# mueller-franzes/medfusion

Hardware: AMD Instinct MI355X
Metric: images/sec at 256x256, 150 DDIM steps (DiffusionPipeline.sample incl. VAE decode) (higher is better)
Workload: dtype f32 (emulated: fp16 pairs -- 23-bit operands, and 23-bit STORAGE of the tensors between the UNet's conv blocks: they exist as fp16 pairs only)

## Files before the change

medfusion_amd/csrc/groupnorm.hip:

```cpp
#include "common.h"
#include <stdlib.h>
#include "gn_partial.h"

using namespace mf;

namespace {

__global__ __launch_bounds__(256) void gn_stats_final_kernel(const double* __restrict__ partial, float* __restrict__ stats, int NG, int G, int chunks,
                                                              double count, float eps) {
  const int t = blockIdx.x * blockDim.x + threadIdx.x;
  const int i = t >> 4, l = t & 15;
  double s = 0, q = 0;
  if (i < NG) {
    const int n = i / G, g = i - n * G;
    for (int c = l; c < chunks; c += 16) {
      const double* p = partial + (((long)n * chunks + c) * G + g) * 2;
      s += p[0]; q += p[1];
    }
  }
#pragma unroll
  for (int off = 8; off > 0; off >>= 1) {
    s += __shfl_xor(s, off, 64);
    q += __shfl_xor(q, off, 64);
  }
// ... 110 lines not shown
    *reinterpret_cast<float4*>(out + i * 4) = make_float4(e[0], e[1], e[2], e[3]);
    store_split4(sp.outs, i * 4, e[0], e[1], e[2], e[3], sc);
  }
}

struct GnChan {
  float mean[4], rstd[4], ga[4], be[4];
  float4 em;
};

__device__ __forceinline__ GnChan gn_chan_consts(const float* sm, const float* __restrict__ gamma, const float* __restrict__ beta,
                                                 const float* __restrict__ emb_row, int c, int cpg) {
  GnChan k;
  if (cpg % 4 == 0) {
    const int g = c / cpg;
#pragma unroll
    for (int i = 0; i < 4; ++i) { k.mean[i] = sm[2 * g]; k.rstd[i] = sm[2 * g + 1]; }
  } else {
#pragma unroll
    for (int i = 0; i < 4; ++i) { const int g = (c + i) / cpg; k.mean[i] = sm[2 * g]; k.rstd[i] = sm[2 * g + 1]; }
  }
  if (gamma) {
    const float4 ga = *reinterpret_cast<const float4*>(gamma + c), be = *reinterpret_cast<const float4*>(beta + c);
    k.ga[0] = ga.x; k.ga[1] = ga.y; k.ga[2] = ga.z; k.ga[3] = ga.w;
    k.be[0] = be.x; k.be[1] = be.y; k.be[2] = be.z; k.be[3] = be.w;
  } else {
#pragma unroll
    for (int i = 0; i < 4; ++i) { k.ga[i] = 1.f; k.be[i] = 0.f; }
  }
  k.em = emb_row ? *reinterpret_cast<const float4*>(emb_row + c) : make_float4(0.f, 0.f, 0.f, 0.f);
  return k;
}

template <bool SPLIT, int U>
__global__ __launch_bounds__(256) void gn_apply_part_kernel(const float* __restrict__ x, const double* __restrict__ partial, int parts, double count, float eps,
                                                            const float* __restrict__ gamma, const float* __restrict__ beta,
                                                            const float* __restrict__ residual, const float* __restrict__ emb, long emb_stride,
                                                            float* __restrict__ out, int HW, int C, int G, int act, const GnSplit sp) {
  __shared__ float sm[2 * 256 + 4];
  __shared__ double sd[2 * 256];
  const int n = blockIdx.y, tid = threadIdx.x;
  const int C4 = C >> 2, cpg = C / G;
  const unsigned per4 = (unsigned)HW * (unsigned)C4;
  const long base = (long)n * per4;
  constexpr unsigned SPAN = 256u * U;
  const unsigned step = gridDim.x * SPAN;
  const bool res_p = SPLIT && sp.res_pairs != nullptr;
  const bool res_f = !res_p && residual != nullptr;
  const bool fixed_c = (256 % C4) == 0;
  const float* emb_row = emb ? emb + (long)n * emb_stride : nullptr;

  float4 v[U], r[U];
  uint2 rh[U], rl[U];
  unsigned jw = blockIdx.x * SPAN;
#define GN_LOAD_ROUND()                                                                                                  \
  _Pragma("unroll") for (int u = 0; u < U; ++u) {                                                                        \
    const unsigned j = jw + 256u * u + tid;                                                                              \
    if (j < per4) {                                                                                                      \
      v[u] = *reinterpret_cast<const float4*>(x + (base + j) * 4);                                                       \
      if (res_p) {                                                                                                       \
        const long e = (base + j) * 4;                                                                                   \
        const uint2* g_ = reinterpret_cast<const uint2*>(reinterpret_cast<const char*>(sp.res_pairs) + (e >> 3) * 32 + ((e >> 2) & 1) * 8); \
        rh[u] = g_[0]; rl[u] = g_[2];                            \
      } else if (res_f) r[u] = *reinterpret_cast<const float4*>(residual + (base + j) * 4);                              \
    }                                                                                                                    \
  }
// ... 37 lines not shown
  }
  GnChan kc = gn_chan_consts(sm, gamma, beta, emb_row, fixed_c ? (tid % C4) * 4 : 0, cpg);

  while (jw < per4) {
#pragma unroll
    for (int u = 0; u < U; ++u) {
      const unsigned j = jw + 256u * u + tid;
      if (j < per4) {
        if (!fixed_c) kc = gn_chan_consts(sm, gamma, beta, emb_row, (int)(j % (unsigned)C4) * 4, cpg);
        float e[4] = {v[u].x, v[u].y, v[u].z, v[u].w};
#pragma unroll
        for (int k = 0; k < 4; ++k) {
          float t = (e[k] - kc.mean[k]) * kc.rstd[k];
          if (gamma) t = t * kc.ga[k] + kc.be[k];
          if (act == 1) t = swish_apply(t);
          e[k] = t;
        }
        if (res_p) {
          const sf_f16x2 h0 = __builtin_bit_cast(sf_f16x2, rh[u].x), h1 = __builtin_bit_cast(sf_f16x2, rh[u].y),
                         l0 = __builtin_bit_cast(sf_f16x2, rl[u].x), l1 = __builtin_bit_cast(sf_f16x2, rl[u].y);
          e[0] += ((float)h0[0] + (float)l0[0] * kLoInv) * rsc; e[1] += ((float)h0[1] + (float)l0[1] * kLoInv) * rsc;
          e[2] += ((float)h1[0] + (float)l1[0] * kLoInv) * rsc; e[3] += ((float)h1[1] + (float)l1[1] * kLoInv) * rsc;
        } else if (res_f) { e[0] += r[u].x; e[1] += r[u].y; e[2] += r[u].z; e[3] += r[u].w; }
        if (emb) { e[0] += kc.em.x; e[1] += kc.em.y; e[2] += kc.em.z; e[3] += kc.em.w; }
        if (!SPLIT || out) *reinterpret_cast<float4*>(out + (base + j) * 4) = make_float4(e[0], e[1], e[2], e[3]);
        if (SPLIT) store_split4<false>(sp.outs, (base + j) * 4, e[0], e[1], e[2], e[3], sc);
      }
    }
    jw += step;
    if (jw < per4) GN_LOAD_ROUND()
  }
#undef GN_LOAD_ROUND
}

__global__ __launch_bounds__(256) void maxabs_kernel(const float* __restrict__ x, float* __restrict__ partial, long per_sample4) {
  const int n = blockIdx.y;
  const float4* p = reinterpret_cast<const float4*>(x) + (long)n * per_sample4;
  float m = 0.f;
  for (long i = (long)blockIdx.x * blockDim.x + threadIdx.x; i < per_sample4; i += (long)gridDim.x * blockDim.x) {
    const float4 v = p[i];
    m = fmaxf(fmaxf(m, fmaxf(fabsf(v.x), fabsf(v.y))), fmaxf(fabsf(v.z), fabsf(v.w)));
  }
  m = wave_max(m);
  if ((threadIdx.x & 63) == 0) partial[((long)n * gridDim.x + blockIdx.x) * 4 + (threadIdx.x >> 6)] = m;
}

__global__ __launch_bounds__(64) void bound_finalize_kernel(const float* __restrict__ partial, float* __restrict__ bound, int slots) {
  const int n = blockIdx.x;
  float m = 0.f;
  for (int i = threadIdx.x; i < slots; i += 64) m = fmaxf(m, partial[(long)n * slots + i]);
  m = wave_max(m);
  if (threadIdx.x == 0) bound[n] = m;
}

}

extern "C" {

size_t mf_gn_stats_workspace_bytes(int N, int HW, int C, int G) {
  if (N <= 0 || HW <= 0 || G <= 0) return 0;
  return (size_t)N * stats_chunks(HW) * G * 2 * sizeof(double);
}

int mf_gn_stats_f32(const float* x, float* stats, void* workspace, size_t workspace_bytes, int N, int HW, int C, int G, float eps,
                    void* stream) {
  MF_REQUIRE(x && stats && N > 0 && HW > 0 && C > 0 && G > 0, MF_EINVAL, "gn_stats: bad args");
// ... 58 lines not shown
                                  int C, int G, int act, void* stream) {
  return mf_gn_apply_from_partials_pairs_f32(x, gn_partial, parts, eps, gamma, beta, residual, nullptr, emb, emb_stride, out, out_split, res_bound,
                                             res_bound_slots, res_nslots, emb_bound, bconst, out_bound, N, HW, C, G, act, stream);
}

int mf_gn_apply_from_partials_pairs_f32(const float* x, const double* gn_partial, int parts, float eps, const float* gamma, const float* beta,
                                        const float* residual, const void* residual_pairs, const float* emb, int64_t emb_stride, float* out,
                                        void* out_split, const float* res_bound, const float* res_bound_slots, int res_nslots,
                                        const float* emb_bound, float bconst, float* out_bound, int N, int HW, int C, int G, int act, void* stream) {
  MF_REQUIRE(x && (out || out_split) && gn_partial && parts > 0 && N > 0 && N <= 65535 && HW > 0 && C > 0, MF_EINVAL, "gn_apply_from_partials: bad args");
  MF_REQUIRE(!residual_pairs || (!residual && out_split && res_bound), MF_EINVAL,
             "gn_apply_from_partials: a residual given as fp16 pairs needs out_split and the res_bound that scaled it, and excludes the fp32 residual");
  MF_REQUIRE(G > 0 && G <= 256 && C % G == 0 && C % 4 == 0, MF_EUNSUPPORTED, "gn_apply_from_partials: C=%d G=%d (C %% 4 == 0, C %% G == 0, G <= 256)", C, G);
  MF_REQUIRE(!out_split || (C % 8 == 0 && out_bound), MF_EUNSUPPORTED, "gn_apply_from_partials: the fp16-pair output needs C %% 8 == 0 and out_bound");
  MF_REQUIRE(!out_split || !residual || res_bound || (res_bound_slots && res_nslots > 0), MF_EINVAL,
             "gn_apply_from_partials: the fp16-pair output needs res_bound (or res_bound_slots) with a residual");
  MF_REQUIRE(!out_split || !emb || emb_bound, MF_EINVAL, "gn_apply_from_partials: the fp16-pair output needs emb_bound with an embedding");
  MF_REQUIRE((gamma == nullptr) == (beta == nullptr), MF_EINVAL, "gn_apply_from_partials: gamma/beta must both be given or both NULL");
  MF_REQUIRE(!emb || emb_stride % 4 == 0, MF_EUNSUPPORTED, "gn_apply_from_partials: emb_stride must be a multiple of 4");
  hipStream_t s = (hipStream_t)stream;
  const long per4 = (long)HW * (C / 4);
  const double nelem = (double)N * HW * C;
  ProfScope ps(MF_FAM_GN_APPLY, s, 8.0 * nelem, 4.0 * nelem * (1 + (out ? 1 : 0) + (residual || residual_pairs ? 1 : 0) + (out_split ? 1 : 0)));
  MF_REQUIRE(per4 < (1L << 31), MF_EUNSUPPORTED, "gn_apply_from_partials: %ld float4 per sample", per4);
  const long total_blocks = ((long)N * per4 + 255) / 256;
  static const int force_u = [] { const char* e = getenv("MF_GN_U"); const int v = e ? atoi(e) : 0; return (v == 1 || v == 2 || v == 4) ? v : 0; }();
  const int U = force_u ? force_u : total_blocks >= 4 * 1024 ? 4 : total_blocks >= 2 * 1024 ? 2 : 1;
  long bps = (per4 + 256 * U - 1) / (256 * U);
  static const int per_cu = [] { const char* e = getenv("MF_GN_BLOCKS_PER_CU"); const int v = e ? atoi(e) : 8; return v < 1 ? 1 : v > 32 ? 32 : v; }();
  const long cap = (256 * per_cu + N - 1) / N;
  if (bps > cap) bps = cap;
  const GnSplit sp{out_split, nullptr, res_bound, emb_bound, bconst, out_bound, res_bound ? nullptr : res_bound_slots, res_nslots, residual_pairs};
  const double count = (double)HW * (C / G);
#define GN_PART_LAUNCH(SPLIT_, U_)                                                                                                          \
  MF_LAUNCH((gn_apply_part_kernel<SPLIT_, U_>), dim3((int)bps, N), dim3(256), 0, s, x, gn_partial, parts, count, eps, gamma, beta, residual, emb, \
            (long)emb_stride, out, HW, C, G, act, sp)
  if (out_split) {
    if (U == 4) GN_PART_LAUNCH(true, 4); else if (U == 2) GN_PART_LAUNCH(true, 2); else GN_PART_LAUNCH(true, 1);
  } else {
    if (U == 4) GN_PART_LAUNCH(false, 4); else if (U == 2) GN_PART_LAUNCH(false, 2); else GN_PART_LAUNCH(false, 1);
  }
#undef GN_PART_LAUNCH
  return check_launch("gn_apply_from_partials");
}

int mf_maxabs_rows_slots(int64_t per_row) {
  const long p4 = per_row / 4;
  int blocks = (int)((p4 + 1023) / 1024);
  if (blocks > 64) blocks = 64;
  if (blocks < 1) blocks = 1;
  return blocks * 4;
}

int mf_maxabs_rows_f32(const float* x, float* partial, float* bound, int N, int64_t per_row, void* stream) {
  MF_REQUIRE(x && partial && N > 0 && per_row > 0 && per_row % 4 == 0 && N <= 65535, MF_EINVAL, "maxabs_rows: bad args (per_row %% 4 == 0)");
  hipStream_t s = (hipStream_t)stream;
  ProfScope ps(MF_FAM_MISC, s, 0, 4.0 * N * (double)per_row);
  const int slots = mf_maxabs_rows_slots(per_row);
  MF_LAUNCH(maxabs_kernel, dim3(slots / 4, N), dim3(256), 0, s, x, partial, (long)(per_row / 4));
  int rc = check_launch("maxabs_rows");
  if (rc || !bound) return rc;
  MF_LAUNCH(bound_finalize_kernel, dim3(N), dim3(64), 0, s, partial, bound, slots);
  return check_launch("bound_finalize");
}

int mf_bound_finalize_f32(const float* partial, float* bound, int N, int slots, void* stream) {
  MF_REQUIRE(partial && bound && N > 0 && slots > 0, MF_EINVAL, "bound_finalize: bad args");
  ProfScope ps(MF_FAM_MISC, (hipStream_t)stream, 0, 4.0 * N * slots);
  MF_LAUNCH(bound_finalize_kernel, dim3(N), dim3(64), 0, (hipStream_t)stream, partial, bound, slots);
  return check_launch("bound_finalize");
}


int mf_gn_partial_parts(int HW) { return HW > 0 ? stats_chunks(HW) : 0; }

// ... 24 lines not shown
```

medfusion_amd/csrc/split_f16.h:

```cpp
#pragma once
#include <hip/hip_runtime.h>

namespace mf {

typedef float sf_f32x4 __attribute__((ext_vector_type(4)));
typedef unsigned int sf_u32x4 __attribute__((ext_vector_type(4)));
typedef unsigned int sf_u32x2 __attribute__((ext_vector_type(2)));
typedef _Float16 sf_f16x2 __attribute__((ext_vector_type(2)));

constexpr float kLoScale = 2048.f, kLoInv = 1.f / 2048.f, kF16Max = 65504.f;

__device__ __forceinline__ int scale_exp_of(float bound) {
  const int e = (int)((__float_as_uint(bound) >> 23) & 0xffu) - 127;
  const int s = e - 14;
  return s < -100 ? -100 : (s > 100 ? 100 : s);
}
__device__ __forceinline__ float exp2i(int s) { return __uint_as_float((unsigned)(127 + s) << 23); }

__device__ __forceinline__ float clamp_f16_range(float a) {
  const float c = __builtin_fminf(__builtin_fmaxf(a, -kF16Max), kF16Max);
  return __builtin_fabsf(a) <= 3.4028234663852886e38f ? c : a;
}
template <bool CLAMP = true>
__device__ __forceinline__ void split2_f16(float a, float b, unsigned& hi, unsigned& lo) {
  if (CLAMP) {
    a = clamp_f16_range(a);
    b = clamp_f16_range(b);
  }
  const _Float16 ha = (_Float16)a, hb = (_Float16)b;
  const float ra = (a - (float)ha) * kLoScale, rb = (b - (float)hb) * kLoScale;
  const sf_f16x2 h = {ha, hb}, l = {(_Float16)ra, (_Float16)rb};
  hi = __builtin_bit_cast(unsigned, h);
  lo = __builtin_bit_cast(unsigned, l);
}
template <bool CLAMP = true>
__device__ __forceinline__ void split8_f16(const sf_f32x4 v0, const sf_f32x4 v1, sf_u32x4& hi, sf_u32x4& lo) {
  const float a0 = v0[0], a1 = v0[1], a2 = v0[2], a3 = v0[3], b0 = v1[0], b1 = v1[1], b2 = v1[2], b3 = v1[3];
  unsigned h0, h1, h2, h3, l0, l1, l2, l3;
  split2_f16<CLAMP>(a0, a1, h0, l0);
  split2_f16<CLAMP>(a2, a3, h1, l1);
  split2_f16<CLAMP>(b0, b1, h2, l2);
  split2_f16<CLAMP>(b2, b3, h3, l3);
  hi = sf_u32x4{h0, h1, h2, h3};
// ... 29 lines not shown
```

medfusion_amd/csrc/winograd.h:

```cpp
#pragma once
#include "common.h"
#include "split_f16.h"

namespace mfw {
using namespace mf;
typedef float wf32x4 __attribute__((ext_vector_type(4)));

__global__ __launch_bounds__(256) void wino_pack_weight_kernel(const float* __restrict__ w, float* __restrict__ u, long n) {
  const long i = (long)blockIdx.x * 256 + threadIdx.x;
  if (i >= n) return;
  double g[3][3], t[4][3];
#pragma unroll
  for (int r = 0; r < 3; ++r)
#pragma unroll
    for (int c = 0; c < 3; ++c) g[r][c] = (double)w[i * 9 + r * 3 + c];
#pragma unroll
  for (int c = 0; c < 3; ++c) {
    t[0][c] = g[0][c];
    t[1][c] = 0.5 * (g[0][c] + g[1][c] + g[2][c]);
    t[2][c] = 0.5 * (g[0][c] - g[1][c] + g[2][c]);
    t[3][c] = g[2][c];
  }
#pragma unroll
  for (int r = 0; r < 4; ++r) {
// ... 7 lines not shown

__device__ __forceinline__ float4 wino_load_pairs4(const void* pairs, long e) {
  const uint2* g = reinterpret_cast<const uint2*>(reinterpret_cast<const char*>(pairs) + (e >> 3) * 32 + ((e >> 2) & 1) * 8);
  const uint2 h = g[0], l = g[2];
  const sf_f16x2 h0 = __builtin_bit_cast(sf_f16x2, h.x), h1 = __builtin_bit_cast(sf_f16x2, h.y), l0 = __builtin_bit_cast(sf_f16x2, l.x),
                 l1 = __builtin_bit_cast(sf_f16x2, l.y);
  return make_float4((float)h0[0] + (float)l0[0] * kLoInv, (float)h0[1] + (float)l0[1] * kLoInv, (float)h1[0] + (float)l1[0] * kLoInv,
                     (float)h1[1] + (float)l1[1] * kLoInv);
}

__device__ __forceinline__ void wino_bt_d_b(float* d) {
#pragma unroll
  for (int c = 0; c < 4; ++c) {
    const float d0 = d[c], d1 = d[4 + c], d2 = d[8 + c], d3 = d[12 + c];
    d[c] = d0 - d2; d[4 + c] = d1 + d2; d[8 + c] = d2 - d1; d[12 + c] = d1 - d3;
  }
#pragma unroll
  for (int r = 0; r < 4; ++r) {
    const float t0 = d[4 * r], t1 = d[4 * r + 1], t2 = d[4 * r + 2], t3 = d[4 * r + 3];
    d[4 * r] = t0 - t2; d[4 * r + 1] = t1 + t2; d[4 * r + 2] = t2 - t1; d[4 * r + 3] = t1 - t3;
  }
}

__global__ __launch_bounds__(256) void wino_input_kernel(const void* __restrict__ xs, const float* __restrict__ xbound, void* __restrict__ vs,
                                                          float* __restrict__ vbound, int N, int H, int W, int C) {
  const int C4 = C >> 2, TW = W >> 1, T = (H >> 1) * TW;
  const long total = (long)N * T * C4, stride = (long)gridDim.x * 256;
  const long plane = (long)N * T * C;
  for (long i = (long)blockIdx.x * 256 + threadIdx.x; i < total; i += stride) {
    const int c4 = (int)(i % C4);
    const long r = i / C4;
    const int tile = (int)(r % T), n = (int)(r / T);
    const int ty = tile / TW, tx = tile - ty * TW;
    const float b = xbound ? xbound[n] : 0.f;
    const float vb = 4.f * b;
    const float f = xbound ? exp2i(scale_exp_of(b)) * exp2i(-scale_exp_of(vb)) : 1.f;
    float d[4][16];
#pragma unroll
    for (int py = 0; py < 4; ++py)
#pragma unroll
      for (int px = 0; px < 4; ++px) {
        const int y = 2 * ty - 1 + py, x = 2 * tx - 1 + px;
        float4 v = make_float4(0.f, 0.f, 0.f, 0.f);
        if ((unsigned)y < (unsigned)H && (unsigned)x < (unsigned)W) v = wino_load_pairs4(xs, (((long)n * H + y) * W + x) * C + c4 * 4);
        d[0][4 * py + px] = v.x; d[1][4 * py + px] = v.y; d[2][4 * py + px] = v.z; d[3][4 * py + px] = v.w;
      }
#pragma unroll
    for (int k = 0; k < 4; ++k) wino_bt_d_b(d[k]);
    const long e0 = ((long)n * T + tile) * C + c4 * 4;
#pragma unroll
    for (int k = 0; k < 16; ++k) store_split4<true>(vs, (long)k * plane + e0, d[0][k], d[1][k], d[2][k], d[3][k], f);
    if (vbound && tile == 0 && c4 == 0) {
#pragma unroll
      for (int k = 0; k < 16; ++k) vbound[k * N + n] = vb;
    }
  }
}

__global__ __launch_bounds__(256) void wino_input_f32_kernel(const float* __restrict__ x, float* __restrict__ v, int N, int H, int W, int C) {
  const int C4 = C >> 2, TW = W >> 1, T = (H >> 1) * TW;
  const long total = (long)N * T * C4, stride = (long)gridDim.x * 256;
  const long plane = (long)N * T * C;
  for (long i = (long)blockIdx.x * 256 + threadIdx.x; i < total; i += stride) {
    const int c4 = (int)(i % C4);
    const long r = i / C4;
    const int tile = (int)(r % T), n = (int)(r / T);
    const int ty = tile / TW, tx = tile - ty * TW;
    float d[4][16];
#pragma unroll
    for (int py = 0; py < 4; ++py)
#pragma unroll
      for (int px = 0; px < 4; ++px) {
        const int y = 2 * ty - 1 + py, xx = 2 * tx - 1 + px;
        float4 q = make_float4(0.f, 0.f, 0.f, 0.f);
        if ((unsigned)y < (unsigned)H && (unsigned)xx < (unsigned)W) q = *reinterpret_cast<const float4*>(x + (((long)n * H + y) * W + xx) * C + c4 * 4);
        d[0][4 * py + px] = q.x; d[1][4 * py + px] = q.y; d[2][4 * py + px] = q.z; d[3][4 * py + px] = q.w;
      }
#pragma unroll
    for (int k = 0; k < 4; ++k) wino_bt_d_b(d[k]);
// ... 91 lines not shown
  void* out_pairs;
  float* out_bound;
  void* out_wino;
  float* wino_bound;
  int N, H, W, C, G, act;
  float eps, bconst;
  int v_nt;
  int v_f32;
  int xcd_map;
};

__device__ __forceinline__ float wino_pair_round(float a) {
  const _Float16 h = (_Float16)a;
  const _Float16 l = (_Float16)((a - (float)h) * kLoScale);
  return (float)h + (float)l * kLoInv;
}

__global__ __launch_bounds__(256) void wino_tail_kernel(const WinoTailP p) {
  extern __shared__ __attribute__((aligned(16))) float ys[];
  __shared__ double sd[8];
  __shared__ float sf[8];
  const int tid = threadIdx.x, lane = tid & 63, wave = tid >> 6;
  int lin = blockIdx.x;
  if (p.xcd_map) {
    const int total = p.G * p.N, q = total >> 3, r = total & 7, xcd = lin & 7, within = lin >> 3;
    lin = (xcd < r ? xcd * (q + 1) : r * (q + 1) + (xcd - r) * q) + within;
  }
  const int g = lin % p.G, n = lin / p.G;
  const int C = p.C, cpg = C / p.G, cq = cpg >> 2, c0 = g * cpg;
  const int H = p.H, W = p.W, HW = H * W, TW = W >> 1, T = (H >> 1) * TW;
  const long plane = (long)p.N * T * C;
  const int c4 = tid % cq;
  constexpr int RJ = 4;
  uint2 rph[RJ], rpl[RJ];
  float4 rpf[RJ];
#pragma unroll
  for (int j = 0; j < RJ; ++j) {
    rph[j] = make_uint2(0u, 0u); rpl[j] = make_uint2(0u, 0u); rpf[j] = make_float4(0.f, 0.f, 0.f, 0.f);
    const int it = tid + 256 * j;
    if (it < HW * cq) {
      const long eo = ((long)n * HW + it / cq) * C + c0 + c4 * 4;
      if (p.res_pairs) {
        const uint2* gp = reinterpret_cast<const uint2*>(reinterpret_cast<const char*>(p.res_pairs) + (eo >> 3) * 32 + ((eo >> 2) & 1) * 8);
        rph[j] = gp[0]; rpl[j] = gp[2];
      } else if (p.res_f32) {
        rpf[j] = *reinterpret_cast<const float4*>(p.res_f32 + eo);
      }
    }
  }
  const float4 b4 = p.bias ? *reinterpret_cast<const float4*>(p.bias + c0 + c4 * 4) : make_float4(0.f, 0.f, 0.f, 0.f);
  double s = 0, q = 0;
  for (int it = tid; it < T * cq; it += 256) {
    const int t = it / cq;
    const float* src = p.m + ((long)n * T + t) * C + c0 + c4 * 4;
    float4 v[16];
#pragma unroll
    for (int k = 0; k < 16; ++k) v[k] = *reinterpret_cast<const float4*>(src + (long)k * plane);
    float4 o[4];
#pragma unroll
    for (int e = 0; e < 4; ++e) {
      float mm[16];
#pragma unroll
      for (int k = 0; k < 16; ++k) mm[k] = e == 0 ? v[k].x : e == 1 ? v[k].y : e == 2 ? v[k].z : v[k].w;
      float a0[4], a1[4];
#pragma unroll
      for (int c = 0; c < 4; ++c) {
        a0[c] = (mm[c] + mm[4 + c]) + mm[8 + c];
        a1[c] = (mm[4 + c] - mm[8 + c]) - mm[12 + c];
      }
      const float be = e == 0 ? b4.x : e == 1 ? b4.y : e == 2 ? b4.z : b4.w;
      const float y00 = ((a0[0] + a0[1]) + a0[2]) + be, y01 = ((a0[1] - a0[2]) - a0[3]) + be;
      const float y10 = ((a1[0] + a1[1]) + a1[2]) + be, y11 = ((a1[1] - a1[2]) - a1[3]) + be;
      if (e == 0) { o[0].x = y00; o[1].x = y01; o[2].x = y10; o[3].x = y11; }
      if (e == 1) { o[0].y = y00; o[1].y = y01; o[2].y = y10; o[3].y = y11; }
      if (e == 2) { o[0].z = y00; o[1].z = y01; o[2].z = y10; o[3].z = y11; }
      if (e == 3) { o[0].w = y00; o[1].w = y01; o[2].w = y10; o[3].w = y11; }
    }
    const int ty = t / TW, tx = t - ty * TW;
    float* dst = ys + ((2 * ty) * W + 2 * tx) * cpg + c4 * 4;
    *reinterpret_cast<float4*>(dst) = o[0];
    *reinterpret_cast<float4*>(dst + cpg) = o[1];
    *reinterpret_cast<float4*>(dst + W * cpg) = o[2];
    *reinterpret_cast<float4*>(dst + W * cpg + cpg) = o[3];
    float s1 = 0.f, s2 = 0.f;
#pragma unroll
    for (int j = 0; j < 4; ++j) {
      s1 += (o[j].x + o[j].y) + (o[j].z + o[j].w);
      s2 = fmaf(o[j].x, o[j].x, s2); s2 = fmaf(o[j].y, o[j].y, s2); s2 = fmaf(o[j].z, o[j].z, s2); s2 = fmaf(o[j].w, o[j].w, s2);
    }
    s += (double)s1;
    q += (double)s2;
  }
#pragma unroll
  for (int off = 32; off > 0; off >>= 1) {
    s += __shfl_xor(s, off, 64);
    q += __shfl_xor(q, off, 64);
  }
  if (lane == 0) { sd[wave] = s; sd[4 + wave] = q; }
  if (p.res_slots) {
    float mx = 0.f;
    for (int i = tid; i < p.res_nslots; i += 256) mx = fmaxf(mx, p.res_slots[(long)n * p.res_nslots + i]);
    mx = wave_max(mx);
    if (lane == 0) sf[wave] = mx;
  }
  __syncthreads();
  const double S = ((sd[0] + sd[1]) + sd[2]) + sd[3], Q = ((sd[4] + sd[5]) + sd[6]) + sd[7];
  const double count = (double)HW * cpg;
  const double mean_d = S / count;
  double var = Q / count - mean_d * mean_d;
  if (var < 0) var = 0;
  const float mean = (float)mean_d, rstd = (float)(1.0 / sqrt(var + (double)p.eps));
  const float rb = p.res_slots ? fmaxf(fmaxf(sf[0], sf[1]), fmaxf(sf[2], sf[3])) : (p.res_bound ? p.res_bound[n] : 0.f);
  const float ob = p.bconst + rb + (p.emb_bound ? p.emb_bound[n] : 0.f);
  const float osc = exp2i(-scale_exp_of(ob));
  const float rsc = p.res_pairs ? exp2i(scale_exp_of(p.res_bound[n])) : 1.f;
  const float vb = 4.f * ob;
  if (g == 0) {
    if (tid == 0 && p.out_bound) p.out_bound[n] = ob;
    if (tid < 16 && p.wino_bound) p.wino_bound[tid * p.N + n] = vb;
  }
  float ga[4] = {1.f, 1.f, 1.f, 1.f}, be[4] = {0.f, 0.f, 0.f, 0.f};
  if (p.gamma) {
    const float4 g4 = *reinterpret_cast<const float4*>(p.gamma + c0 + c4 * 4), e4 = *reinterpret_cast<const float4*>(p.beta + c0 + c4 * 4);
    ga[0] = g4.x; ga[1] = g4.y; ga[2] = g4.z; ga[3] = g4.w;
    be[0] = e4.x; be[1] = e4.y; be[2] = e4.z; be[3] = e4.w;
  }
  const float4 em = p.emb ? *reinterpret_cast<const float4*>(p.emb + (long)n * p.emb_stride + c0 + c4 * 4) : make_float4(0.f, 0.f, 0.f, 0.f);
  const bool keep = p.out_wino != nullptr;
  auto pairs_to_f4 = [](uint2 h, uint2 l) {
    const sf_f16x2 h0 = __builtin_bit_cast(sf_f16x2, h.x), h1 = __builtin_bit_cast(sf_f16x2, h.y), l0 = __builtin_bit_cast(sf_f16x2, l.x),
                   l1 = __builtin_bit_cast(sf_f16x2, l.y);
    return make_float4((float)h0[0] + (float)l0[0] * kLoInv, (float)h0[1] + (float)l0[1] * kLoInv, (float)h1[0] + (float)l1[0] * kLoInv,
                       (float)h1[1] + (float)l1[1] * kLoInv);
  };
#define WINO_TAIL_ELEMENT(IT, RES_EXPR_PAIRS, RES_EXPR_F32)                                                            \
  {                                                                                                                   \
    const int pix = (IT) / cq;                                                                                        \
    float* yp = ys + pix * cpg + c4 * 4;                                                                              \
    const float4 v = *reinterpret_cast<const float4*>(yp);                                                            \
    float e[4] = {v.x, v.y, v.z, v.w};                                                                                \
    _Pragma("unroll") for (int k = 0; k < 4; ++k) {                                                                   \
      float t = (e[k] - mean) * rstd;                                                                                 \
      if (p.gamma) t = t * ga[k] + be[k];                                                                             \
      if (p.act == 1) t = swish_apply(t);                                                                             \
      e[k] = t;                                                                                                       \
    }                                                                                                                 \
    const long eo = ((long)n * HW + pix) * C + c0 + c4 * 4;                                                           \
    if (p.res_pairs) {                                                                                                \
      const float4 r = RES_EXPR_PAIRS;                                                                                \
      e[0] += r.x * rsc; e[1] += r.y * rsc; e[2] += r.z * rsc; e[3] += r.w * rsc;                                     \
    } else if (p.res_f32) {                                                                                           \
      const float4 r = RES_EXPR_F32;                                                                                  \
      e[0] += r.x; e[1] += r.y; e[2] += r.z; e[3] += r.w;                                                             \
    }                                                                                                                 \
    if (p.emb) { e[0] += em.x; e[1] += em.y; e[2] += em.z; e[3] += em.w; }                                            \
    if (p.out_f32) *reinterpret_cast<float4*>(p.out_f32 + eo) = make_float4(e[0], e[1], e[2], e[3]);                  \
    if (p.out_pairs) store_split4<false>(p.out_pairs, eo, e[0], e[1], e[2], e[3], osc);    \
    if (keep) *reinterpret_cast<float4*>(yp) = p.v_f32 ? make_float4(e[0], e[1], e[2], e[3])                                                                     \
                                                       : make_float4(wino_pair_round(e[0] * osc), wino_pair_round(e[1] * osc), wino_pair_round(e[2] * osc), wino_pair_round(e[3] * osc)); \
  }
#pragma unroll
  for (int j = 0; j < RJ; ++j) {
    const int it = tid + 256 * j;
    if (it < HW * cq) WINO_TAIL_ELEMENT(it, pairs_to_f4(rph[j], rpl[j]), rpf[j])
  }
  for (int it = tid + 256 * RJ; it < HW * cq; it += 256) WINO_TAIL_ELEMENT(it, wino_load_pairs4(p.res_pairs, eo), *reinterpret_cast<const float4*>(p.res_f32 + eo))
#undef WINO_TAIL_ELEMENT
  if (!keep) return;
  __syncthreads();
  const float f = exp2i(scale_exp_of(ob)) * exp2i(-scale_exp_of(vb));
  for (int it = tid; it < T * cq; it += 256) {
    const int t = it / cq, ty = t / TW, tx = t - ty * TW;
    float d[4][16];
#pragma unroll
    for (int py = 0; py < 4; ++py)
#pragma unroll
      for (int px = 0; px < 4; ++px) {
        const int y = 2 * ty - 1 + py, x = 2 * tx - 1 + px;
        float4 v = make_float4(0.f, 0.f, 0.f, 0.f);
        if ((unsigned)y < (unsigned)H && (unsigned)x < (unsigned)W) v = *reinterpret_cast<const float4*>(ys + (y * W + x) * cpg + c4 * 4);
        d[0][4 * py + px] = v.x; d[1][4 * py + px] = v.y; d[2][4 * py + px] = v.z; d[3][4 * py + px] = v.w;
      }
#pragma unroll
    for (int k = 0; k < 4; ++k) wino_bt_d_b(d[k]);
    const long e0 = ((long)n * T + t) * C + c0 + c4 * 4;
    if (p.v_f32) {
#pragma unroll
      for (int k = 0; k < 16; ++k)
        __builtin_nontemporal_store(wf32x4{d[0][k], d[1][k], d[2][k], d[3][k]}, reinterpret_cast<wf32x4*>(reinterpret_cast<float*>(p.out_wino) + (long)k * plane + e0));
    } else if (p.v_nt) {
#pragma unroll
      for (int k = 0; k < 16; ++k) store_split4<true, true>(p.out_wino, (long)k * plane + e0, d[0][k], d[1][k], d[2][k], d[3][k], f);
    } else {
#pragma unroll
      for (int k = 0; k < 16; ++k) store_split4<true>(p.out_wino, (long)k * plane + e0, d[0][k], d[1][k], d[2][k], d[3][k], f);
    }
  }
}

}
```

Baseline: 40.57.

## Hoist and prefetch residual/param loads in GroupNorm apply and Winograd tail kernels

Adds a new code path, on by default, in the GroupNorm apply kernel, the Winograd input transform and the fused GN/Winograd tail. It issues the activation, residual, gamma/beta, embedding and bound loads unconditionally before the statistics reduction, using a zero buffer in place of null pointers, and pins them in registers with asm barriers. The tail residual loop is software-pipelined one element ahead, with output-mode specialisation, and fixed-channel handling becomes a template parameter. A lighter LDS-only barrier replaces __syncthreads. The aim is to overlap global-memory latency with the reduction and remove branchy dependent loads, at the cost of more register pressure and some redundant loads.

```diff
diff --git a/medfusion_amd/csrc/groupnorm.hip b/medfusion_amd/csrc/groupnorm.hip
--- a/medfusion_amd/csrc/groupnorm.hip
+++ b/medfusion_amd/csrc/groupnorm.hip
@@ -166,6 +166,163 @@
   return k;
 }
 
+#if MF_PASS_CHAIN == 2
+__device__ __forceinline__ GnChan gn_chan_consts_any(const float* sm, const float* __restrict__ gamma, const float* __restrict__ beta,
+                                                     const float* __restrict__ emb_row, int c, int cpg) {
+  GnChan k;
+  const float4 ga = *reinterpret_cast<const float4*>(gamma ? gamma + c : kZeros8), be = *reinterpret_cast<const float4*>(gamma ? beta + c : kZeros8);
+  k.em = *reinterpret_cast<const float4*>(emb_row ? emb_row + c : kZeros8);
+  k.ga[0] = ga.x; k.ga[1] = ga.y; k.ga[2] = ga.z; k.ga[3] = ga.w;
+  k.be[0] = be.x; k.be[1] = be.y; k.be[2] = be.z; k.be[3] = be.w;
+  if (cpg % 4 == 0) {
+    const int g = c / cpg;
+#pragma unroll
+    for (int i = 0; i < 4; ++i) { k.mean[i] = sm[2 * g]; k.rstd[i] = sm[2 * g + 1]; }
+  } else {
+#pragma unroll
+    for (int i = 0; i < 4; ++i) { const int g = (c + i) / cpg; k.mean[i] = sm[2 * g]; k.rstd[i] = sm[2 * g + 1]; }
+  }
+  return k;
+}
+
+template <bool SPLIT, int U, bool FIXED_C>
+__global__ __launch_bounds__(256) void gn_apply_part_kernel(const float* __restrict__ x, const double* __restrict__ partial, int parts, double count, float eps,
+                                                            const float* __restrict__ gamma, const float* __restrict__ beta,
+                                                            const float* __restrict__ residual, const float* __restrict__ emb, long emb_stride,
+                                                            float* __restrict__ out, int HW, int C, int G, int act, const GnSplit sp) {
+  __shared__ float sm[2 * 256 + 4];
+  __shared__ double sd[2 * 256];
+  const int n = blockIdx.y, tid = threadIdx.x;
+  const int C4 = C >> 2, cpg = C / G;
+  const unsigned per4 = (unsigned)HW * (unsigned)C4;
+  const long base = (long)n * per4;
+  constexpr unsigned SPAN = 256u * U;
+  const unsigned step = gridDim.x * SPAN;
+  const bool res_p = SPLIT && sp.res_pairs != nullptr;
+  const bool res_f = !res_p && residual != nullptr;
+  constexpr bool fixed_c = FIXED_C;
+  const float* emb_row = emb ? emb + (long)n * emb_stride : nullptr;
+  const int PPT = 256 / G, g = tid % G, kk = tid / G;
+
+  const double* rp0 = partial + (((long)n * parts + min(kk, parts - 1)) * G + g) * 2;
+  const double rec_s = rp0[0], rec_q = rp0[1];
+  float rbv = 0.f, ebv = 0.f, sl0 = 0.f;
+  if (SPLIT) {
+    rbv = *(sp.res_bound ? sp.res_bound + n : kZeros8);
+    ebv = *(sp.emb_bound ? sp.emb_bound + n : kZeros8);
+    sl0 = *((sp.res_slots && sp.res_nslots > 0) ? sp.res_slots + (long)n * sp.res_nslots + min(tid, sp.res_nslots - 1) : kZeros8);
+  }
+  const int cfix = fixed_c ? (tid % C4) * 4 : 0;
+  float4 g4 = *reinterpret_cast<const float4*>(gamma ? gamma + cfix : kZeros8), e4 = *reinterpret_cast<const float4*>(gamma ? beta + cfix : kZeros8);
+  float4 em4 = *reinterpret_cast<const float4*>(emb_row ? emb_row + cfix : kZeros8);
+  const char* const rbase = res_p ? reinterpret_cast<const char*>(sp.res_pairs) : res_f ? reinterpret_cast<const char*>(residual) : reinterpret_cast<const char*>(kZeros8);
+  const int rhalf = res_p ? 16 : 8;
+  float4 v[U];
+  uint2 ra[U], rb[U];
+  unsigned jw = blockIdx.x * SPAN;
+#define GN_LOAD_ROUND()                                                                                                  \
+  _Pragma("unroll") for (int u = 0; u < U; ++u) {                                                                        \
+    const long e = (base + min(jw + 256u * u + tid, per4 - 1u)) * 4;                                                     \
+    v[u] = *reinterpret_cast<const float4*>(x + e);                                                                      \
+    const char* q_ = rbase + (res_p ? (e >> 3) * 32 + ((e >> 2) & 1) * 8 : res_f ? e * 4 : 0L);                          \
+    ra[u] = *reinterpret_cast<const uint2*>(q_);                                                                         \
+    rb[u] = *reinterpret_cast<const uint2*>(q_ + rhalf);    \
+  }
+  GN_LOAD_ROUND()
+
+  {
+    double s = 0, q = 0;
+    if (kk < PPT) {
+      if (kk < parts) { s += rec_s; q += rec_q; }
+      for (int k = kk + PPT; k < parts; k += PPT) {
+        const double* p = partial + (((long)n * parts + k) * G + g) * 2;
+        s += p[0]; q += p[1];
+      }
+    }
+    sd[tid] = s; sd[256 + tid] = q;
+  }
+  if (SPLIT && sp.res_slots) {
+    float m = fmaxf(0.f, sl0);
+    for (int i = tid + 256; i < sp.res_nslots; i += 256) m = fmaxf(m, sp.res_slots[(long)n * sp.res_nslots + i]);
+    m = wave_max(m);
+    if ((tid & 63) == 0) sm[2 * 256 + (tid >> 6)] = m;
+  }
+  MF_LDS_BARRIER();
+  if (tid < G) {
+    double s = sd[tid], q = sd[256 + tid];
+    for (int k2 = 1; k2 < PPT; ++k2) { s += sd[k2 * G + tid]; q += sd[256 + k2 * G + tid]; }
+    const double mean = s / count;
+    double var = q / count - mean * mean;
+    if (var < 0) var = 0;
+    sm[2 * tid] = (float)mean;
+    sm[2 * tid + 1] = (float)(1.0 / sqrt(var + (double)eps));
+  }
+  MF_LDS_BARRIER();
+  float sc = 1.f, rsc = 1.f, obound = 0.f;
+  if (SPLIT) {
+    const float rbd = sp.res_slots ? fmaxf(fmaxf(sm[512], sm[513]), fmaxf(sm[514], sm[515])) : rbv;
+    obound = sp.bconst + rbd + ebv;
+    sc = exp2i(-scale_exp_of(obound));
+    if (res_p) rsc = exp2i(scale_exp_of(rbv));
+  }
+  GnChan kc;
+  {
+    if (cpg % 4 == 0) {
+      const int gq = cfix / cpg;
+#pragma unroll
+      for (int i = 0; i < 4; ++i) { kc.mean[i] = sm[2 * gq]; kc.rstd[i] = sm[2 * gq + 1]; }
+    } else {
+#pragma unroll
+      for (int i = 0; i < 4; ++i) { const int gq = (cfix + i) / cpg; kc.mean[i] = sm[2 * gq]; kc.rstd[i] = sm[2 * gq + 1]; }
+    }
+    asm volatile("" : "+v"(g4.x), "+v"(g4.y), "+v"(g4.z), "+v"(g4.w), "+v"(e4.x), "+v"(e4.y), "+v"(e4.z), "+v"(e4.w), "+v"(em4.x), "+v"(em4.y), "+v"(em4.z), "+v"(em4.w));
+    kc.ga[0] = g4.x; kc.ga[1] = g4.y; kc.ga[2] = g4.z; kc.ga[3] = g4.w;
+    kc.be[0] = e4.x; kc.be[1] = e4.y; kc.be[2] = e4.z; kc.be[3] = e4.w;
+    kc.em = em4;
+  }
+
+  for (;;) {
+#pragma unroll
+    for (int u = 0; u < U; ++u)
+      asm volatile("" : "+v"(v[u].x), "+v"(v[u].y), "+v"(v[u].z), "+v"(v[u].w), "+v"(ra[u].x), "+v"(ra[u].y), "+v"(rb[u].x), "+v"(rb[u].y));
+#pragma unroll
+    for (int u = 0; u < U; ++u) {
+      const unsigned j = jw + 256u * u + tid;
+      if (j < per4) {
+        if (!fixed_c) {
+          kc = gn_chan_consts_any(sm, gamma, beta, emb_row, (int)(j % (unsigned)C4) * 4, cpg);
+          asm volatile("" : "+v"(kc.ga[0]), "+v"(kc.ga[1]), "+v"(kc.ga[2]), "+v"(kc.ga[3]), "+v"(kc.be[0]), "+v"(kc.be[1]), "+v"(kc.be[2]), "+v"(kc.be[3]),
+                            "+v"(kc.em.x), "+v"(kc.em.y), "+v"(kc.em.z), "+v"(kc.em.w));
+        }
+        float e[4] = {v[u].x, v[u].y, v[u].z, v[u].w};
+#pragma unroll
+        for (int k = 0; k < 4; ++k) {
+          float t = (e[k] - kc.mean[k]) * kc.rstd[k];
+          if (gamma) t = t * kc.ga[k] + kc.be[k];
+          if (act == 1) t = swish_apply(t);
+          e[k] = t;
+        }
+        if (res_p) {
+          const sf_f16x2 h0 = __builtin_bit_cast(sf_f16x2, ra[u].x), h1 = __builtin_bit_cast(sf_f16x2, ra[u].y),
+                         l0 = __builtin_bit_cast(sf_f16x2, rb[u].x), l1 = __builtin_bit_cast(sf_f16x2, rb[u].y);
+          e[0] += ((float)h0[0] + (float)l0[0] * kLoInv) * rsc; e[1] += ((float)h0[1] + (float)l0[1] * kLoInv) * rsc;
+          e[2] += ((float)h1[0] + (float)l1[0] * kLoInv) * rsc; e[3] += ((float)h1[1] + (float)l1[1] * kLoInv) * rsc;
+        } else if (res_f) {
+          e[0] += __uint_as_float(ra[u].x); e[1] += __uint_as_float(ra[u].y); e[2] += __uint_as_float(rb[u].x); e[3] += __uint_as_float(rb[u].y);
+        }
+        if (emb) { e[0] += kc.em.x; e[1] += kc.em.y; e[2] += kc.em.z; e[3] += kc.em.w; }
+        if (!SPLIT || out) *reinterpret_cast<float4*>(out + (base + j) * 4) = make_float4(e[0], e[1], e[2], e[3]);
+        if (SPLIT) store_split4<false>(sp.outs, (base + j) * 4, e[0], e[1], e[2], e[3], sc);
+      }
+    }
+    jw += step;
+    if (jw >= per4) break;
+    GN_LOAD_ROUND()
+  }
+#undef GN_LOAD_ROUND
+  if (SPLIT && blockIdx.x == 0 && tid == 0) sp.out_bound[n] = obound;
+}
+#else
 template <bool SPLIT, int U>
 __global__ __launch_bounds__(256) void gn_apply_part_kernel(const float* __restrict__ x, const double* __restrict__ partial, int parts, double count, float eps,
                                                             const float* __restrict__ gamma, const float* __restrict__ beta,
@@ -269,6 +426,7 @@
   }
 #undef GN_LOAD_ROUND
 }
+#endif
 
 __global__ __launch_bounds__(256) void maxabs_kernel(const float* __restrict__ x, float* __restrict__ partial, long per_sample4) {
   const int n = blockIdx.y;
@@ -393,15 +551,26 @@
   if (bps > cap) bps = cap;
   const GnSplit sp{out_split, nullptr, res_bound, emb_bound, bconst, out_bound, res_bound ? nullptr : res_bound_slots, res_nslots, residual_pairs};
   const double count = (double)HW * (C / G);
+#if MF_PASS_CHAIN == 2
+#define GN_PART_LAUNCH_(SPLIT_, U_, FIXED_)                                                                                                          \
+  MF_LAUNCH((gn_apply_part_kernel<SPLIT_, U_, FIXED_>), dim3((int)bps, N), dim3(256), 0, s, x, gn_partial, parts, count, eps, gamma, beta, residual, \
+            emb, (long)emb_stride, out, HW, C, G, act, sp)
+#define GN_PART_LAUNCH(SPLIT_, U_)                                                    \
+  do {                                                                                \
+    if (256 % (C / 4) == 0) GN_PART_LAUNCH_(SPLIT_, U_, true); else GN_PART_LAUNCH_(SPLIT_, U_, false); \
+  } while (0)
+#else
 #define GN_PART_LAUNCH(SPLIT_, U_)                                                                                                          \
   MF_LAUNCH((gn_apply_part_kernel<SPLIT_, U_>), dim3((int)bps, N), dim3(256), 0, s, x, gn_partial, parts, count, eps, gamma, beta, residual, emb, \
             (long)emb_stride, out, HW, C, G, act, sp)
+#endif
   if (out_split) {
     if (U == 4) GN_PART_LAUNCH(true, 4); else if (U == 2) GN_PART_LAUNCH(true, 2); else GN_PART_LAUNCH(true, 1);
   } else {
     if (U == 4) GN_PART_LAUNCH(false, 4); else if (U == 2) GN_PART_LAUNCH(false, 2); else GN_PART_LAUNCH(false, 1);
   }
 #undef GN_PART_LAUNCH
+#undef GN_PART_LAUNCH_
   return check_launch("gn_apply_from_partials");
 }
 
diff --git a/medfusion_amd/csrc/split_f16.h b/medfusion_amd/csrc/split_f16.h
--- a/medfusion_amd/csrc/split_f16.h
+++ b/medfusion_amd/csrc/split_f16.h
@@ -9,6 +9,17 @@
 typedef _Float16 sf_f16x2 __attribute__((ext_vector_type(2)));
 
 constexpr float kLoScale = 2048.f, kLoInv = 1.f / 2048.f, kF16Max = 65504.f;
+
+#ifndef MF_PASS_CHAIN
+#define MF_PASS_CHAIN 2
+#endif
+__attribute__((unused, aligned(16))) static __device__ float kZeros8[8] = {0.f, 0.f, 0.f, 0.f, 0.f, 0.f, 0.f, 0.f};
+#define MF_LDS_BARRIER()                                  \
+  do {                                                    \
+    asm volatile("s_waitcnt lgkmcnt(0)" ::: "memory");    \
+    __builtin_amdgcn_s_barrier();                         \
+    asm volatile("" ::: "memory");                        \
+  } while (0)
 
 __device__ __forceinline__ int scale_exp_of(float bound) {
   const int e = (int)((__float_as_uint(bound) >> 23) & 0xffu) - 127;
diff --git a/medfusion_amd/csrc/winograd.h b/medfusion_amd/csrc/winograd.h
--- a/medfusion_amd/csrc/winograd.h
+++ b/medfusion_amd/csrc/winograd.h
@@ -63,6 +63,34 @@
     const long r = i / C4;
     const int tile = (int)(r % T), n = (int)(r / T);
     const int ty = tile / TW, tx = tile - ty * TW;
+#if MF_PASS_CHAIN == 2
+    const float b = *(xbound ? xbound + n : kZeros8);
+    uint2 ph[16], pl[16];
+#pragma unroll
+    for (int py = 0; py < 4; ++py)
+#pragma unroll
+      for (int px = 0; px < 4; ++px) {
+        const int y = min(max(2 * ty - 1 + py, 0), H - 1), x = min(max(2 * tx - 1 + px, 0), W - 1);
+        const long e = (((long)n * H + y) * W + x) * C + c4 * 4;
+        const uint2* gp = reinterpret_cast<const uint2*>(reinterpret_cast<const char*>(xs) + (e >> 3) * 32 + ((e >> 2) & 1) * 8);
+        ph[4 * py + px] = gp[0]; pl[4 * py + px] = gp[2];
+      }
+    const float vb = 4.f * b;
+    const float f = xbound ? exp2i(scale_exp_of(b)) * exp2i(-scale_exp_of(vb)) : 1.f;
+    float d[4][16];
+#pragma unroll
+    for (int py = 0; py < 4; ++py)
+#pragma unroll
+      for (int px = 0; px < 4; ++px) {
+        const int y = 2 * ty - 1 + py, x = 2 * tx - 1 + px, k = 4 * py + px;
+        const bool inside = (unsigned)y < (unsigned)H && (unsigned)x < (unsigned)W;
+        const uint2 h = inside ? ph[k] : make_uint2(0u, 0u), l = inside ? pl[k] : make_uint2(0u, 0u);
+        const sf_f16x2 h0 = __builtin_bit_cast(sf_f16x2, h.x), h1 = __builtin_bit_cast(sf_f16x2, h.y), l0 = __builtin_bit_cast(sf_f16x2, l.x),
+                       l1 = __builtin_bit_cast(sf_f16x2, l.y);
+        d[0][k] = (float)h0[0] + (float)l0[0] * kLoInv; d[1][k] = (float)h0[1] + (float)l0[1] * kLoInv;
+        d[2][k] = (float)h1[0] + (float)l1[0] * kLoInv; d[3][k] = (float)h1[1] + (float)l1[1] * kLoInv;
+      }
+#else
     const float b = xbound ? xbound[n] : 0.f;
     const float vb = 4.f * b;
     const float f = xbound ? exp2i(scale_exp_of(b)) * exp2i(-scale_exp_of(vb)) : 1.f;
@@ -76,6 +104,7 @@
         if ((unsigned)y < (unsigned)H && (unsigned)x < (unsigned)W) v = wino_load_pairs4(xs, (((long)n * H + y) * W + x) * C + c4 * 4);
         d[0][4 * py + px] = v.x; d[1][4 * py + px] = v.y; d[2][4 * py + px] = v.z; d[3][4 * py + px] = v.w;
       }
+#endif
 #pragma unroll
     for (int k = 0; k < 4; ++k) wino_bt_d_b(d[k]);
     const long e0 = ((long)n * T + tile) * C + c4 * 4;
@@ -233,6 +262,29 @@
   const long plane = (long)p.N * T * C;
   const int c4 = tid % cq;
   constexpr int RJ = 4;
+#if MF_PASS_CHAIN == 2
+  const int nel = HW * cq, cc = c0 + c4 * 4;
+  const bool res_p = p.res_pairs != nullptr, res_f = !res_p && p.res_f32 != nullptr;
+  const char* const rbase = res_p ? reinterpret_cast<const char*>(p.res_pairs) : res_f ? reinterpret_cast<const char*>(p.res_f32) : reinterpret_cast<const char*>(kZeros8);
+  const int rhalf = res_p ? 16 : 8;
+  auto res_at = [&](int it) {
+    const long eo = ((long)n * HW + it / cq) * C + cc;
+    return rbase + (res_p ? (eo >> 3) * 32 + ((eo >> 2) & 1) * 8 : res_f ? eo * 4 : 0L);
+  };
+  uint2 rqa[RJ + 1], rqb[RJ + 1];
+#pragma unroll
+  for (int j = 0; j <= RJ; ++j) {
+    const char* q = res_at(min(tid + 256 * j, nel - 1));
+    rqa[j] = *reinterpret_cast<const uint2*>(q);
+    rqb[j] = *reinterpret_cast<const uint2*>(q + rhalf);
+  }
+  float4 b4 = *reinterpret_cast<const float4*>(p.bias ? p.bias + cc : kZeros8);
+  float4 g4 = *reinterpret_cast<const float4*>(p.gamma ? p.gamma + cc : kZeros8), e4 = *reinterpret_cast<const float4*>(p.gamma ? p.beta + cc : kZeros8);
+  float4 em = *reinterpret_cast<const float4*>(p.emb ? p.emb + (long)n * p.emb_stride + cc : kZeros8);
+  const float rbv = *(p.res_bound ? p.res_bound + n : kZeros8), ebv = *(p.emb_bound ? p.emb_bound + n : kZeros8);
+  const bool slots = p.res_slots != nullptr && p.res_nslots > 0;
+  float sl0 = *(slots ? p.res_slots + (long)n * p.res_nslots + min(tid, p.res_nslots - 1) : kZeros8);
+#else
   uint2 rph[RJ], rpl[RJ];
   float4 rpf[RJ];
 #pragma unroll
@@ -250,6 +302,7 @@
     }
   }
   const float4 b4 = p.bias ? *reinterpret_cast<const float4*>(p.bias + c0 + c4 * 4) : make_float4(0.f, 0.f, 0.f, 0.f);
+#endif
   double s = 0, q = 0;
   for (int it = tid; it < T * cq; it += 256) {
     const int t = it / cq;
@@ -298,6 +351,15 @@
     q += __shfl_xor(q, off, 64);
   }
   if (lane == 0) { sd[wave] = s; sd[4 + wave] = q; }
+#if MF_PASS_CHAIN == 2
+  if (p.res_slots) {
+    float mx = fmaxf(0.f, sl0);
+    for (int i = tid + 256; i < p.res_nslots; i += 256) mx = fmaxf(mx, p.res_slots[(long)n * p.res_nslots + i]);
+    mx = wave_max(mx);
+    if (lane == 0) sf[wave] = mx;
+  }
+  MF_LDS_BARRIER();
+#else
   if (p.res_slots) {
     float mx = 0.f;
     for (int i = tid; i < p.res_nslots; i += 256) mx = fmaxf(mx, p.res_slots[(long)n * p.res_nslots + i]);
@@ -305,21 +367,34 @@
     if (lane == 0) sf[wave] = mx;
   }
   __syncthreads();
+#endif
   const double S = ((sd[0] + sd[1]) + sd[2]) + sd[3], Q = ((sd[4] + sd[5]) + sd[6]) + sd[7];
   const double count = (double)HW * cpg;
   const double mean_d = S / count;
   double var = Q / count - mean_d * mean_d;
   if (var < 0) var = 0;
   const float mean = (float)mean_d, rstd = (float)(1.0 / sqrt(var + (double)p.eps));
+#if MF_PASS_CHAIN == 2
+  const float rb = p.res_slots ? fmaxf(fmaxf(sf[0], sf[1]), fmaxf(sf[2], sf[3])) : rbv;
+  const float ob = p.bconst + rb + ebv;
+  const float rsc = p.res_pairs ? exp2i(scale_exp_of(rbv)) : 1.f;
+#else
   const float rb = p.res_slots ? fmaxf(fmaxf(sf[0], sf[1]), fmaxf(sf[2], sf[3])) : (p.res_bound ? p.res_bound[n] : 0.f);
   const float ob = p.bconst + rb + (p.emb_bound ? p.emb_bound[n] : 0.f);
+  const float rsc = p.res_pairs ? exp2i(scale_exp_of(p.res_bound[n])) : 1.f;
+#endif
   const float osc = exp2i(-scale_exp_of(ob));
-  const float rsc = p.res_pairs ? exp2i(scale_exp_of(p.res_bound[n])) : 1.f;
   const float vb = 4.f * ob;
   if (g == 0) {
     if (tid == 0 && p.out_bound) p.out_bound[n] = ob;
     if (tid < 16 && p.wino_bound) p.wino_bound[tid * p.N + n] = vb;
   }
+#if MF_PASS_CHAIN == 2
+  asm volatile("" : "+v"(g4.x), "+v"(g4.y), "+v"(g4.z), "+v"(g4.w), "+v"(e4.x), "+v"(e4.y), "+v"(e4.z), "+v"(e4.w), "+v"(em.x), "+v"(em.y), "+v"(em.z), "+v"(em.w));
+#pragma unroll
+  for (int j = 0; j <= RJ; ++j) asm volatile("" : "+v"(rqa[j].x), "+v"(rqa[j].y), "+v"(rqb[j].x), "+v"(rqb[j].y));
+  const float ga[4] = {g4.x, g4.y, g4.z, g4.w}, be[4] = {e4.x, e4.y, e4.z, e4.w};
+#else
   float ga[4] = {1.f, 1.f, 1.f, 1.f}, be[4] = {0.f, 0.f, 0.f, 0.f};
   if (p.gamma) {
     const float4 g4 = *reinterpret_cast<const float4*>(p.gamma + c0 + c4 * 4), e4 = *reinterpret_cast<const float4*>(p.beta + c0 + c4 * 4);
@@ -327,6 +402,7 @@
     be[0] = e4.x; be[1] = e4.y; be[2] = e4.z; be[3] = e4.w;
   }
   const float4 em = p.emb ? *reinterpret_cast<const float4*>(p.emb + (long)n * p.emb_stride + c0 + c4 * 4) : make_float4(0.f, 0.f, 0.f, 0.f);
+#endif
   const bool keep = p.out_wino != nullptr;
   auto pairs_to_f4 = [](uint2 h, uint2 l) {
     const sf_f16x2 h0 = __builtin_bit_cast(sf_f16x2, h.x), h1 = __builtin_bit_cast(sf_f16x2, h.y), l0 = __builtin_bit_cast(sf_f16x2, l.x),
@@ -334,7 +410,8 @@
     return make_float4((float)h0[0] + (float)l0[0] * kLoInv, (float)h0[1] + (float)l0[1] * kLoInv, (float)h1[0] + (float)l1[0] * kLoInv,
                        (float)h1[1] + (float)l1[1] * kLoInv);
   };
-#define WINO_TAIL_ELEMENT(IT, RES_EXPR_PAIRS, RES_EXPR_F32)                                                            \
+#define WINO_TAIL_ELEMENT(IT, RES_EXPR_PAIRS, RES_EXPR_F32) WINO_TAIL_ELEMENT_TO(IT, RES_EXPR_PAIRS, RES_EXPR_F32, p.out_f32, p.out_pairs)
+#define WINO_TAIL_ELEMENT_TO(IT, RES_EXPR_PAIRS, RES_EXPR_F32, TO_F32, TO_PAIRS)                                       \
   {                                                                                                                   \
     const int pix = (IT) / cq;                                                                                        \
     float* yp = ys + pix * cpg + c4 * 4;                                                                              \
@@ -355,20 +432,51 @@
       e[0] += r.x; e[1] += r.y; e[2] += r.z; e[3] += r.w;                                                             \
     }                                                                                                                 \
     if (p.emb) { e[0] += em.x; e[1] += em.y; e[2] += em.z; e[3] += em.w; }                                            \
-    if (p.out_f32) *reinterpret_cast<float4*>(p.out_f32 + eo) = make_float4(e[0], e[1], e[2], e[3]);                  \
-    if (p.out_pairs) store_split4<false>(p.out_pairs, eo, e[0], e[1], e[2], e[3], osc);    \
+    if (TO_F32) *reinterpret_cast<float4*>(p.out_f32 + eo) = make_float4(e[0], e[1], e[2], e[3]);                     \
+    if (TO_PAIRS) store_split4<false>(p.out_pairs, eo, e[0], e[1], e[2], e[3], osc);    \
     if (keep) *reinterpret_cast<float4*>(yp) = p.v_f32 ? make_float4(e[0], e[1], e[2], e[3])                                                                     \
                                                        : make_float4(wino_pair_round(e[0] * osc), wino_pair_round(e[1] * osc), wino_pair_round(e[2] * osc), wino_pair_round(e[3] * osc)); \
   }
+#if MF_PASS_CHAIN == 2
+  auto raw_to_f4 = [](uint2 a, uint2 b) { return make_float4(__uint_as_float(a.x), __uint_as_float(a.y), __uint_as_float(b.x), __uint_as_float(b.y)); };
+  uint2 nqa = rqa[RJ], nqb = rqb[RJ];
+#pragma unroll
+  for (int j = 0; j < RJ; ++j) {
+    const int it = tid + 256 * j;
+    if (it < nel) WINO_TAIL_ELEMENT(it, pairs_to_f4(rqa[j], rqb[j]), raw_to_f4(rqa[j], rqb[j]))
+  }
+#define WINO_TAIL_REST(TO_F32, TO_PAIRS)                                                                              \
+  for (int it = tid + 256 * RJ; it < nel; it += 256) {                                                                \
+    const uint2 cqa = nqa, cqb = nqb;                                                                                 \
+    const char* q = res_at(min(it + 256, nel - 1));                                                                   \
+    nqa = *reinterpret_cast<const uint2*>(q);                                                                         \
+    nqb = *reinterpret_cast<const uint2*>(q + rhalf);                                                                 \
+    WINO_TAIL_ELEMENT_TO(it, pairs_to_f4(cqa, cqb), raw_to_f4(cqa, cqb), TO_F32, TO_PAIRS)                            \
+  }
+  if (nel > 256 * RJ) {
+    if (p.out_f32) {
+      if (p.out_pairs) WINO_TAIL_REST(true, true) else WINO_TAIL_REST(true, false)
+    } else {
+      if (p.out_pairs) WINO_TAIL_REST(false, true) else WINO_TAIL_REST(false, false)
+    }
+  }
+#undef WINO_TAIL_REST
+#else
 #pragma unroll
   for (int j = 0; j < RJ; ++j) {
     const int it = tid + 256 * j;
     if (it < HW * cq) WINO_TAIL_ELEMENT(it, pairs_to_f4(rph[j], rpl[j]), rpf[j])
   }
   for (int it = tid + 256 * RJ; it < HW * cq; it += 256) WINO_TAIL_ELEMENT(it, wino_load_pairs4(p.res_pairs, eo), *reinterpret_cast<const float4*>(p.res_f32 + eo))
+#endif
 #undef WINO_TAIL_ELEMENT
+#undef WINO_TAIL_ELEMENT_TO
   if (!keep) return;
+#if MF_PASS_CHAIN == 2
+  MF_LDS_BARRIER();
+#else
   __syncthreads();
+#endif
   const float f = exp2i(scale_exp_of(ob)) * exp2i(-scale_exp_of(vb));
   for (int it = tid; it < T * cq; it += 256) {
     const int t = it / cq, ty = t / TW, tx = t - ty * TW;
```

Result: faster. 41.28 (median of 6 runs) (+1.7%).
